# srsampson/SingleCarrier

Measured on NVIDIA B200. Metric: demodulated_msym_per_s, higher is better.
Workload: dtype f32

## Files before the change

### include/singlecarrier_b200.h

```cpp
#ifndef SINGLECARRIER_B200_H
#define SINGLECARRIER_B200_H

#include <stddef.h>
#include <stdint.h>

#ifdef __cplusplus
extern "C" {
#endif

#define SC_FRAME_SIZE        1880
#define SC_SYMBOLS_PER_FRAME 376
#define SC_PREAMBLE_LENGTH   128
#define SC_DATA_SYMBOLS      31
#define SC_BITS_PER_CALL     62
#define SC_NTAPS             49
#define SC_EQ_LENGTH         5
#define SC_PACKET_SYMBOLS    376

#define SC_OK        0
#define SC_EINVAL   -1
#define SC_ECUDA    -2
#define SC_ENOMEM   -3
#define SC_ESTATE   -4

// ... 8 lines not shown
    float    max_value;
    float    cost;
    int16_t  max_index;
    int16_t  matches;
    int16_t  rx_timing;
    uint8_t  valid;
    uint8_t  reserved0;
    uint32_t call_index;
    uint32_t reserved1;
} sc_frame_result;


int  sc_create(sc_modem **out, int device, int64_t n_streams, uint32_t flags, float foffset_hz);
void sc_destroy(sc_modem *m);
int  sc_reset(sc_modem *m);
int64_t  sc_n_streams(const sc_modem *m);
uint32_t sc_call_index(const sc_modem *m);
const char *sc_last_error(void);
const char *sc_version(void);
int  sc_device_count(void);
uint64_t sc_launch_count(void);

#define SC_OPT_SLAB_PARTS 1
#define SC_OPT_PROFILE    2
#define SC_OPT_H2D_MODE   3
#define SC_H2D_COLUMNS    0
#define SC_H2D_ROWS       1
#define SC_H2D_FULL       2
#define SC_H2D_COLUMNS_3D 3
#define SC_OPT_FE_SEARCH     4
#define SC_FE_SEARCH_DIRECT  0
#define SC_FE_SEARCH_MMA     1
#define SC_FE_SEARCH_TCGEN05 2
#define SC_OPT_TRACKER       5
#define SC_TRACKER_AUTO      0
#define SC_TRACKER_THREAD    1
#define SC_TRACKER_COOP      2
#define SC_TRACKER_COOP_MAX  1024
#define SC_OPT_OVERLAP       6
#define SC_OVERLAP_AUTO      0
#define SC_OVERLAP_OFF       1
#define SC_OVERLAP_ON        2
#define SC_OVERLAP_MAX       32768
int  sc_set_option(sc_modem *m, int option, int64_t value);
int  sc_profile_read(sc_modem *m, double out[4]);
int  sc_transfer_bytes(const sc_modem *m, uint64_t out[2]);
int  sc_release_caches(void);


int64_t sc_state_size(const sc_modem *m);
int  sc_state_export(sc_modem *m, void *buf, int64_t buf_bytes);
int  sc_state_import(sc_modem *m, const void *buf, int64_t buf_bytes);


int sc_rx_frames_dev(sc_modem *m, const int16_t *in, int64_t stream_stride, int n_frames,
                     sc_frame_result *results, int64_t result_stride, float *eq_dbg, void *stream);
int sc_rx_frames_host(sc_modem *m, const int16_t *in, int64_t stream_stride, int n_frames,
                      sc_frame_result *results, int64_t result_stride, float *eq_dbg);

int sc_rx_frames_soft_dev(sc_modem *m, const int16_t *in, int64_t stream_stride, int n_frames,
                          sc_frame_result *results, int64_t result_stride, float *symbols, void *stream);
int sc_rx_frames_soft_host(sc_modem *m, const int16_t *in, int64_t stream_stride, int n_frames,
                           sc_frame_result *results, int64_t result_stride, float *symbols);


typedef struct {
// ... 132 lines not shown
```

### singlecarrier_b200/csrc/sc_api.cu

```cuda
#include <math.h>
#include <stdarg.h>
#include <stdio.h>
#include <stdlib.h>
#include <string.h>

#include <algorithm>
#include <atomic>
#include <map>
#include <tuple>
#include <mutex>
#include <new>
#include <vector>

#include <nvtx3/nvToolsExt.h>

#include "sc_kernels.h"
#include "sc_common.cuh"

namespace sc {
std::atomic<unsigned long long> g_launch_count{0};
}

struct NvtxRange {
    explicit NvtxRange(const char *name) { nvtxRangePushA(name); }
// ... 58 lines not shown
    cudaEvent_t ev_tab1 = nullptr, ev_tab2 = nullptr;
    int tab_split = 0;
    std::vector<cudaEvent_t> ev_tabc;

    int16_t *stage_in[N_PIPE] = {};
    sc_frame_result *stage_res[N_PIPE] = {};
    float *stage_eq[N_PIPE] = {};
    float *stage_sym[N_PIPE] = {};
    size_t stage_in_cap = 0, stage_res_cap = 0, stage_eq_cap = 0, stage_sym_cap = 0;

    bool packet = false;
    int16_t *pk_hist2 = nullptr;
    float2 *pk_mix_hist2 = nullptr;
    int *pk_t_before[N_PIPE] = {}, *pk_t_at[N_PIPE] = {};
    int2 *pk_list[N_PIPE] = {};
    int *pk_count[N_PIPE] = {};
    float2 *pk_sym[N_PIPE] = {};
    cudaStream_t pk_stream[N_PIPE] = {};
    cudaEvent_t pk_ev_go[N_PIPE] = {}, pk_ev_done[N_PIPE] = {};
    size_t pk_slab_cap = 0;
    unsigned long long *pk_n_host_dev = nullptr;
    sc_packet_result *pk_stage = nullptr;
    size_t pk_stage_cap = 0;
    float2 *pk_sym_stage = nullptr;
    size_t pk_sym_stage_cap = 0;
    PacketKey pk_key;

    bool poisoned = false;
    bool in_flight = false;
    uint64_t h2d_bytes = 0, d2h_bytes = 0;

    int h2d_mode = SC_H2D_COLUMNS;
    const void *search_a_table = nullptr;
    bool fe_search_mma = false;
    bool fe_search_umma = false;
    const void *search_umma_master = nullptr;
    int slab_parts = 0;
    bool profile = false;
    int tracker = SC_TRACKER_AUTO;

    int overlap = SC_OVERLAP_AUTO;
    float2 *ov_win[OV_RING] = {};
    int *ov_max_index[OV_RING] = {};
    float *ov_max_value[OV_RING] = {};
    float *ov_state[OV_RING] = {};
    int *ov_timing[OV_RING] = {};
    cudaStream_t ov_stream[N_PIPE] = {}, ov_data[N_PIPE][2] = {};
    cudaEvent_t ov_ev_fe[N_PIPE][OV_RING] = {}, ov_ev_train[N_PIPE][OV_RING] = {}, ov_ev_data[N_PIPE][OV_RING] = {};
    cudaEvent_t ov_ev_first[N_PIPE] = {}, ov_join[N_PIPE][3] = {};
    bool ov_ready = false;
    std::vector<cudaEvent_t> ev_fe, ev_tk;
};

static inline unsigned lfsr_step(uint16_t &m) {
    unsigned out = ((m >> 1) ^ m) & 1u;
    m = (uint16_t) ((m >> 1) | (out << 14));
    return out;
}
static uint64_t keystream_next_word(uint16_t &m) {
    uint64_t w = 0;
    for (int j = 0; j < SC_BITS_PER_CALL; j++) w |= (uint64_t) lfsr_step(m) << j;
    return w;
}

static uint16_t lfsr_at_call(uint32_t call_index) {
    uint16_t m = 0x4A80;
    const uint32_t steps = (uint32_t) (((uint64_t) call_index * SC_BITS_PER_CALL) % 32767u);
    for (uint32_t k = 0; k < steps; k++) lfsr_step(m);
// ... 72 lines not shown
    if (const char *e = getenv("SC_OVERLAP")) m->overlap = std::max(0, std::min(atoi(e), (int) SC_OVERLAP_ON));
    m->rx_rect = nco_rect(-1100.0f + foffset_hz);
    m->tx_rect = nco_rect(1100.0f);
    int rc = SC_OK;
    auto body = [&]() -> int {
        CU(cudaSetDevice(device));
        const int64_t np = m->n_pad;
        CU(cudaMalloc(&m->timing[0], np * sizeof(int)));
        CU(cudaMalloc(&m->timing[1], np * sizeof(int)));
        CU(cudaMalloc(&m->timing_cold, np * sizeof(int)));
        {
            std::vector<int> t(np, 3);
            CU(cudaMemcpy(m->timing_cold, t.data(), np * sizeof(int), cudaMemcpyHostToDevice));
        }
        CU(cudaMalloc(&m->win, (size_t) (np / 32) * WIN_ROWS * 32 * sizeof(float2)));
        CU(cudaMalloc(&m->max_index, np * sizeof(int)));
        CU(cudaMalloc(&m->max_value, np * sizeof(float)));
        CU(cudaMalloc(&m->hist, (size_t) m->n * FRAME * sizeof(int16_t)));
        CU(cudaMemset(m->hist, 0, (size_t) m->n * FRAME * sizeof(int16_t)));
        CU(cudaMalloc(&m->rx_phase, sizeof(float2)));
        if (m->packet) {
            CU(cudaMalloc(&m->pk_hist2, (size_t) m->n * FRAME * sizeof(int16_t)));
            CU(cudaMemset(m->pk_hist2, 0, (size_t) m->n * FRAME * sizeof(int16_t)));
            CU(cudaMalloc(&m->pk_mix_hist2, (size_t) FRAME * sizeof(float2)));
            CU(cudaMemset(m->pk_mix_hist2, 0, (size_t) FRAME * sizeof(float2)));
            CU(cudaMalloc(&m->pk_n_host_dev, sizeof(unsigned long long)));
        }
        CU(cudaMalloc(&m->unit_phase, sizeof(float2)));
        {
            const float2 one = make_float2(1.0f, 0.0f);
            CU(cudaMemcpy(m->unit_phase, &one, sizeof one, cudaMemcpyHostToDevice));
        }
        if (const char *e = getenv("SC_FE_SEARCH")) {
            m->fe_search_umma = strcmp(e, "tcgen05") == 0;
            m->fe_search_mma = m->fe_search_umma || strcmp(e, "mma") == 0;
        }
        if (const char *e = getenv("SC_H2D_MODE")) m->h2d_mode = std::max(0, std::min(atoi(e), (int) SC_H2D_COLUMNS_3D));
        for (int i = 0; i < N_PIPE; i++) {
            CU(cudaStreamCreateWithFlags(&m->pipe[i], cudaStreamNonBlocking));
            CU(cudaEventCreateWithFlags(&m->ev_done[i], cudaEventDisableTiming));
        }
        CU(cudaEventCreateWithFlags(&m->ev_start, cudaEventDisableTiming));
        CU(cudaStreamCreateWithFlags(&m->tab_stream, cudaStreamNonBlocking));
        CU(cudaEventCreateWithFlags(&m->ev_tab1, cudaEventDisableTiming));
        CU(cudaEventCreateWithFlags(&m->ev_tab2, cudaEventDisableTiming));
        return modem_cold(m);
    };
    rc = body();
    if (rc != SC_OK) {
        sc_destroy(m);
        return rc;
    }
    *out = m;
    return SC_OK;
}

extern "C" void sc_destroy(sc_modem *m) {
    if (!m) return;
    cudaSetDevice(m->device);
    cudaDeviceSynchronize();
    cudaFree(m->timing[0]);
    cudaFree(m->timing[1]);
    cudaFree(m->timing_cold);
    for (cudaEvent_t e : m->ev_fe) cudaEventDestroy(e);
    for (cudaEvent_t e : m->ev_tk) cudaEventDestroy(e);
    cudaFree(m->win);
    cudaFree(m->max_index);
    cudaFree(m->max_value);
// ... 319 lines not shown
        CU(cudaMemcpy2DAsync(m->hist + (size_t) s0 * FRAME, FRAME * sizeof(int16_t), in + (size_t) (n_frames - 1) * FRAME,
                             (size_t) stride * sizeof(int16_t), FRAME * sizeof(int16_t), (size_t) ns, cudaMemcpyDeviceToDevice, st));
    return SC_OK;
}

static int run_slab(sc_modem *m, cudaStream_t st, int64_t s0, int ns, const int16_t *in, int64_t stride,
                    int n_frames, uint32_t call0, const uint64_t *kw, const float2 *mix0, int slot0,
                    sc_frame_result *results, int64_t result_stride, float *eq_dbg, float *sym, bool save_hist,
                    const PacketSink *pk = nullptr, int pipe = 0) {
    float2 *win = m->win + (size_t) (s0 / 32) * WIN_ROWS * 32;
    int tab_waited = -1;
    PacketSrc psrc;
    int pk_chunk = 0, pk_done = 0;
    if (pk) {
        if (ns > PK_CAP) return fail(SC_ESTATE, "packet mode: slab larger than the packet scratch");
        CU(cudaMemcpyAsync(m->pk_t_before[pipe], m->timing[(call0 + 1) & 1] + s0, (size_t) ns * sizeof(int), cudaMemcpyDeviceToDevice, st));
        CU(cudaMemcpyAsync(m->pk_t_at[pipe], m->timing[call0 & 1] + s0, (size_t) ns * sizeof(int), cudaMemcpyDeviceToDevice, st));
        psrc.results = results;
        psrc.result_stride = result_stride;
        psrc.in = in;
        psrc.stride = stride;
        psrc.hist1 = m->hist + (size_t) s0 * FRAME;
        psrc.hist2 = m->pk_hist2 + (size_t) s0 * FRAME;
        psrc.mix0 = mix0;
        psrc.mix_hist2 = slot0 >= 1 ? mix0 - FRAME : m->pk_mix_hist2;
        psrc.timing_before_call0 = m->pk_t_before[pipe];
        psrc.timing_at_call0 = m->pk_t_at[pipe];
        psrc.call0 = call0;
        psrc.stream0 = (int) s0;
        psrc.wide = m->wide;
        pk_chunk = std::max(1, PK_CAP / ns);
    }
    const bool tracker_coop = m->tracker == SC_TRACKER_COOP || (m->tracker == SC_TRACKER_AUTO && ns <= SC_TRACKER_COOP_MAX);
    const bool plain = !pk && !m->packet && !m->profile && !m->fe_search_mma && !eq_dbg && !m->state_dbg;
    if (plain && n_frames >= 2 && (m->overlap == SC_OVERLAP_ON || (m->overlap == SC_OVERLAP_AUTO && m->n <= SC_OVERLAP_MAX)))
        return run_slab_overlapped(m, st, pipe, s0, ns, in, stride, n_frames, call0, kw, mix0, slot0, results, result_stride,
                                   sym, save_hist, tracker_coop);
    for (int j = 0; j < n_frames; j++) {
        const uint32_t n = call0 + (uint32_t) j;
        int *tc = m->timing[n & 1] + s0, *tn = m->timing[(n + 1) & 1] + s0;
        if (m->profile) CU(prof_mark(m->ev_tk, st));
        {
            NvtxRange range("sc:track_kernel");
            CU(launch_track(m->debug_eq && eq_dbg != nullptr, win, m->max_index + s0, m->max_value + s0, tc, tn,
                            results + j, result_stride, eq_dbg ? eq_dbg + (size_t) j * 10 : nullptr,
                            m->state_dbg ? m->state_dbg + (size_t) s0 * TRACK_STATE_FLOATS : nullptr, n, kw[j], ns, st, tracker_coop,
                            sym ? sym + (size_t) j * SYM_FLOATS : nullptr));
        }
        if (m->profile) CU(prof_mark(m->ev_tk, st));
        if (n >= 1) {
            const int16_t *frame;
            int64_t fstride;
            if (j >= 1) {
                frame = in + (size_t) (j - 1) * FRAME;
                fstride = stride;
            } else {
                frame = m->hist + (size_t) s0 * FRAME;
                fstride = FRAME;
            }
            int rcw = table_wait(m, st, slot0 + j, tab_waited);
            if (rcw != SC_OK) return rcw;
            if (m->profile) CU(prof_mark(m->ev_fe, st));
            {
                NvtxRange range("sc:frontend_kernel");
                if (m->fe_search_umma && frontend_umma_eligible(frame, fstride))
                    CU(launch_frontend_umma(m->wide, frame, fstride, mix0 + (size_t) j * FRAME, tc, tn, win, m->max_index + s0,
                                            m->max_value + s0, ns, st, m->search_umma_master));
                else
                    CU(launch_frontend(m->wide, frame, fstride, mix0 + (size_t) j * FRAME, tc, tn, win, m->max_index + s0,
                                       m->max_value + s0, ns, st,
                                       m->fe_search_mma && !m->fe_search_umma ? m->search_a_table : nullptr));
            }
            if (m->profile) CU(prof_mark(m->ev_fe, st));
        }
        if (pk && (j + 1 - pk_done == pk_chunk || j + 1 == n_frames)) {
            NvtxRange range("sc:packet_pass");
            int rcw = table_wait(m, st, slot0 + j, tab_waited);
            if (rcw != SC_OK) return rcw;
            CU(cudaEventRecord(m->pk_ev_go[pipe], st));
            CU(cudaStreamWaitEvent(m->pk_stream[pipe], m->pk_ev_go[pipe], 0));
            CU(launch_packet_pass(psrc, ns, pk_done, j + 1, PK_CAP, m->pk_list[pipe], m->pk_count[pipe], m->pk_sym[pipe],
                                  m->pk_key, pk->packets, pk->capacity, pk->n_packets, pk->symbols, m->pk_stream[pipe]));
            pk_done = j + 1;
        }
    }
    if (pk) {
        CU(cudaEventRecord(m->pk_ev_done[pipe], m->pk_stream[pipe]));
        CU(cudaStreamWaitEvent(st, m->pk_ev_done[pipe], 0));
    }
    if (m->packet && save_hist && n_frames > 0) {
        if (n_frames >= 2)
            CU(cudaMemcpy2DAsync(m->pk_hist2 + (size_t) s0 * FRAME, FRAME * sizeof(int16_t),
                                 in + (size_t) (n_frames - 2) * FRAME, (size_t) stride * sizeof(int16_t),
                                 FRAME * sizeof(int16_t), (size_t) ns, cudaMemcpyDeviceToDevice, st));
        else
            CU(cudaMemcpyAsync(m->pk_hist2 + (size_t) s0 * FRAME, m->hist + (size_t) s0 * FRAME,
                               (size_t) ns * FRAME * sizeof(int16_t), cudaMemcpyDeviceToDevice, st));
    }
    if (save_hist && n_frames > 0) {
        CU(cudaMemcpy2DAsync(m->hist + (size_t) s0 * FRAME, FRAME * sizeof(int16_t),
                             in + (size_t) (n_frames - 1) * FRAME, (size_t) stride * sizeof(int16_t),
                             FRAME * sizeof(int16_t), (size_t) ns, cudaMemcpyDeviceToDevice, st));
    }
    return SC_OK;
}

static int64_t pick_slab(int64_t n, int64_t lo, int64_t parts) {
    int64_t s = (n + parts - 1) / parts;
    s = std::max<int64_t>(s, lo);
    s = (s + 127) / 128 * 128;
    return s;
}

static int rx_begin(sc_modem *m, const char *who, const int16_t *in, int64_t stream_stride, int n_frames,
                    sc_frame_result *results, int64_t result_stride, float *eq_dbg, std::vector<uint64_t> &kw,
                    uint16_t &lfsr) {
    if (!m || !in || !results || n_frames < 0) return fail(SC_EINVAL, "%s: bad arguments", who);
    if (m->poisoned) return fail(SC_ESTATE, "%s: an earlier batch failed part-way; call sc_reset() first", who);
    if (n_frames == 0) return SC_OK;
    if (stream_stride < (int64_t) n_frames * FRAME || result_stride < n_frames)
        return fail(SC_EINVAL, "%s: stride smaller than the batch", who);
    if (eq_dbg && !m->debug_eq) return fail(SC_EINVAL, "%s: eq_dbg needs SC_FLAG_DEBUG_EQ", who);
    if (m->fe_search_mma) {
        int rc = m->fe_search_umma ? search_umma_master(m->device, &m->search_umma_master)
                                   : search_table(m->device, &m->search_a_table);
        if (rc != SC_OK) return rc;
    }
    lfsr = m->lfsr_rx;
    kw.resize(n_frames);
    for (int j = 0; j < n_frames; j++) kw[j] = keystream_next_word(lfsr);
    return SC_OK;
}

static int rx_end(sc_modem *m, int rc, int n_frames, uint16_t lfsr) {
    if (rc != SC_OK) {
        if (m->in_flight) m->poisoned = true;
        m->in_flight = false;
        return rc;
    }
    m->in_flight = false;
    m->lfsr_rx = lfsr;
    m->call += (uint32_t) n_frames;
    return SC_OK;
}

static int rx_frames_dev_body(sc_modem *m, const int16_t *in, int64_t stream_stride, int n_frames,
                              sc_frame_result *results, int64_t result_stride, float *eq_dbg, float *sym,
                              cudaStream_t user, const uint64_t *kw, const PacketSink *pk = nullptr) {
    CU(cudaSetDevice(m->device));
    CU(cudaEventRecord(m->ev_start, user));
    CU(cudaStreamWaitEvent(m->pipe[0], m->ev_start, 0));
    m->in_flight = true;
    int rc = prepare_tables(m, n_frames, m->pipe[0]);
    if (rc != SC_OK) return rc;
    CU(cudaEventRecord(m->ev_start, m->pipe[0]));
    for (int i = 1; i < N_PIPE; i++) CU(cudaStreamWaitEvent(m->pipe[i], m->ev_start, 0));

    int64_t slab = pick_slab(m->n, m->slab_parts > 0 ? 128 : 8192, m->slab_parts > 0 ? m->slab_parts : 2);
    if (pk) slab = std::min<int64_t>(slab, PK_CAP);
    int k = 0;
// ... 879 lines not shown
    if (h.magic != STATE_MAGIC || h.version != STATE_VERSION) return fail(SC_EINVAL, "sc_state_import: not a state image");
    if (h.n != m->n || h.n_pad != m->n_pad || h.flags != m->flags || h.foffset != m->foffset)
        return fail(SC_EINVAL, "sc_state_import: the image was taken from a bank with other parameters");
    int rc = state_quiesce(m);
    if (rc != SC_OK) return rc;
    if (m->mix_cap < 1) {
        CU(cudaMalloc(&m->mix_table, (size_t) 2 * FRAME * sizeof(float2)));
        m->mix_cap = 1;
    }
    CU(cudaMemcpy(m->rx_phase, &h.rx_phase, sizeof(float2), cudaMemcpyHostToDevice));
    CU(cudaMemcpy(m->timing[h.call & 1], b + L.off_timing, (size_t) m->n_pad * sizeof(int), cudaMemcpyHostToDevice));
    CU(cudaMemcpy(m->max_index, b + L.off_maxi, (size_t) m->n_pad * sizeof(int), cudaMemcpyHostToDevice));
    CU(cudaMemcpy(m->max_value, b + L.off_maxv, (size_t) m->n_pad * sizeof(float), cudaMemcpyHostToDevice));
    CU(cudaMemcpy(m->win, b + L.off_win, (size_t) (m->n_pad / 32) * WIN_ROWS * 32 * sizeof(float2), cudaMemcpyHostToDevice));
    CU(cudaMemcpy(m->hist, b + L.off_hist, (size_t) m->n * FRAME * sizeof(int16_t), cudaMemcpyHostToDevice));
    CU(cudaMemcpy(m->mix_table, b + L.off_mix, (size_t) FRAME * sizeof(float2), cudaMemcpyHostToDevice));
    m->call = h.call;
    m->lfsr_rx = h.lfsr_rx;
    m->poisoned = m->in_flight = false;
    return SC_OK;
}

extern "C" int sc_set_option(sc_modem *m, int option, int64_t value) {
    if (!m) return fail(SC_EINVAL, "sc_set_option: null handle");
    switch (option) {
        case SC_OPT_SLAB_PARTS:
            if (value < 0 || value > 1024) return fail(SC_EINVAL, "sc_set_option: slab parts out of range");
            m->slab_parts = (int) value;
            return SC_OK;
        case SC_OPT_PROFILE:
            m->profile = value != 0;
            return SC_OK;
        case SC_OPT_FE_SEARCH:
            if (value != SC_FE_SEARCH_DIRECT && value != SC_FE_SEARCH_MMA && value != SC_FE_SEARCH_TCGEN05)
                return fail(SC_EINVAL, "sc_set_option: unknown search mode");
            m->fe_search_mma = value != SC_FE_SEARCH_DIRECT;
            m->fe_search_umma = value == SC_FE_SEARCH_TCGEN05;
            return SC_OK;
        case SC_OPT_TRACKER:
            if (value < SC_TRACKER_AUTO || value > SC_TRACKER_COOP) return fail(SC_EINVAL, "sc_set_option: unknown tracker");
            m->tracker = (int) value;
            return SC_OK;
        case SC_OPT_OVERLAP:
            if (value < SC_OVERLAP_AUTO || value > SC_OVERLAP_ON) return fail(SC_EINVAL, "sc_set_option: unknown overlap mode");
            m->overlap = (int) value;
            return SC_OK;
        case SC_OPT_H2D_MODE:
            if (value < SC_H2D_COLUMNS || value > SC_H2D_COLUMNS_3D) return fail(SC_EINVAL, "sc_set_option: unknown H2D mode");
            m->h2d_mode = (int) value;
            return SC_OK;
        default:
            return fail(SC_EINVAL, "sc_set_option: unknown option %d", option);
    }
}

static int prof_sum(std::vector<cudaEvent_t> &v, double *ms, double *count) {
    *ms = 0.0;
    *count = 0.0;
    for (size_t i = 0; i + 1 < v.size(); i += 2) {
        float t = 0.f;
        CU(cudaEventElapsedTime(&t, v[i], v[i + 1]));
        *ms += t;
        *count += 1.0;
    }
    for (cudaEvent_t e : v) cudaEventDestroy(e);
    v.clear();
    return SC_OK;
}

extern "C" int sc_profile_read(sc_modem *m, double out[4]) {
// ... 16 lines not shown
```

### singlecarrier_b200/csrc/sc_frontend_umma.cu

```cuda
#include "sc_common.cuh"
#include "sc_tables.cuh"
#include "sc_frontend.cuh"
#include "sc_umma.cuh"
#include "sc_kernels.h"

#include <stdio.h>
#include <stdlib.h>

namespace sc {

constexpr int FU_WIN = 16;
constexpr int FU_SRCH_WARP0 = FU_WIN, FU_SRCH_WARPS = 4;
constexpr int FU_THREADS = 32 * (FU_WIN + FU_SRCH_WARPS);
constexpr int FU_MIX_BYTES = FE_BUF * 8;
constexpr int FU_W_BYTES = WIN * 8;
static_assert(FU_W_BYTES % 128 == 16 && FU_MIX_BYTES % 16 == 0, "window stride");
constexpr int FU_N = 4 * FU_WIN;
constexpr int FU_KSTEPS = 2 * PRE / 16;
constexpr int FU_B_LBO = (FU_N / 8) * 128;
constexpr int FU_B_BYTES = (2 * PRE / 8) * FU_B_LBO;
constexpr int FU_SBO = 128;
constexpr int FU_A_LBO = ((SU_A_ROWS + 7) / 8) * 128;
constexpr int FU_A_BYTES = 2 * FU_A_LBO;
static_assert(FU_A_BYTES == 16 * SU_A_WORDS4 && FU_A_BYTES % 128 == 0, "master size");
constexpr int FU_TMEM_COLS = FU_N;
constexpr uint32_t FU_IDESC = (1u << 4) | (1u << 7) | (1u << 10) | ((uint32_t) (FU_N >> 3) << 17) | ((128u >> 4) << 24);

struct FuShared {
    unsigned long long a_full;
    unsigned long long tab_full;
    unsigned long long w_full;
    unsigned long long w_empty;
    unsigned long long mma_done;
    uint32_t tmem_base;
    uint32_t warp_max[FU_SRCH_WARPS][FU_WIN];
    float s_abs[FU_WIN];
    int maxidx[FU_WIN];
    int t2[FU_WIN];
    int n_cand[FU_SRCH_WARPS][FU_WIN];
    float ver_v[FU_SRCH_WARPS][FU_WIN];
    int ver_i[FU_SRCH_WARPS][FU_WIN];
    unsigned char cand[FU_SRCH_WARPS][FU_WIN][SM_MAX_CAND];
};
constexpr int FU_OFF_B = FU_A_BYTES;
constexpr int FU_OFF_W = FU_OFF_B + FU_B_BYTES;
constexpr int FU_OFF_MIX = FU_OFF_W + FU_WIN * FU_W_BYTES;
constexpr int FU_TAB_BYTES = FRAME * 8;
constexpr int FU_OFF_TAB = FU_OFF_MIX + FU_WIN * FU_MIX_BYTES;
constexpr int FU_OFF_CTRL = FU_OFF_TAB + FU_TAB_BYTES;
static_assert(FU_OFF_TAB % 16 == 0 && FU_TAB_BYTES % 16 == 0, "TMA bulk copy of the table");
static_assert(FU_OFF_B % 128 == 0 && FU_OFF_W % 128 == 0 && FU_OFF_MIX % 16 == 0 && FU_OFF_CTRL % 16 == 0, "alignment");
constexpr int FU_SMEM = FU_OFF_CTRL + (int) sizeof(FuShared) + 1024;
static_assert(FU_SMEM <= 227 * 1024, "one CTA per SM");

__device__ __forceinline__ void umma_bf16_ss(uint32_t tmem_d, uint64_t a_desc, uint64_t b_desc, uint32_t accumulate) {
    asm volatile(
        "{\n\t.reg .pred p;\n\t"
        "setp.ne.b32 p, %4, 0;\n\t"
        "tcgen05.mma.cta_group::1.kind::f16 [%0], %1, %2, %3, p;\n\t}" ::"r"(tmem_d),
        "l"(a_desc), "l"(b_desc), "r"(FU_IDESC), "r"(accumulate)
        : "memory");
}
__device__ __forceinline__ void fu_tmem_ld16(uint32_t taddr, float (&v)[16]) {
    uint32_t r[16];
    asm volatile(
        "tcgen05.ld.sync.aligned.32x32b.x16.b32 {%0, %1, %2, %3, %4, %5, %6, %7, %8, %9, %10, %11, %12, %13, %14, %15}, [%16];"
        : "=r"(r[0]), "=r"(r[1]), "=r"(r[2]), "=r"(r[3]), "=r"(r[4]), "=r"(r[5]), "=r"(r[6]), "=r"(r[7]), "=r"(r[8]),
          "=r"(r[9]), "=r"(r[10]), "=r"(r[11]), "=r"(r[12]), "=r"(r[13]), "=r"(r[14]), "=r"(r[15])
        : "r"(taddr));
#pragma unroll
    for (int i = 0; i < 16; i++) v[i] = __uint_as_float(r[i]);
}
__device__ __forceinline__ void srch_bar() { asm volatile("bar.sync 1, 128;" ::: "memory"); }

#ifdef FU_PROFILE
#define FU_T(acc) { const long long t_ = clock64(); acc += t_ - t_last; t_last = t_; }
#else
#define FU_T(acc)
#endif

__device__ __forceinline__ int ld_pinned(const int *p) {
    int v;
    asm volatile("ld.global.nc.b32 %0, [%1];" : "=r"(v) : "l"(p));
    return v;
}

template <bool WIDE>
__global__ void __launch_bounds__(FU_THREADS, 1)
frontend_umma_kernel(const int16_t *__restrict__ in, long stream_stride, const float2 *__restrict__ mix_table,
                     const int *__restrict__ timing_cur, const int *__restrict__ timing_next,
                     float2 *__restrict__ win, int *__restrict__ max_index_out, float *__restrict__ max_value_out,
                     int n_streams, const uint4 *__restrict__ a_master) {
    extern __shared__ unsigned char fu_smem_raw[];
    unsigned char *fu_smem = fu_smem_raw + ((1024u - (smem_u32(fu_smem_raw) & 1023u)) & 1023u);
    unsigned char *sA = fu_smem;
    unsigned char *sB = fu_smem + FU_OFF_B;
    unsigned char *sW = fu_smem + FU_OFF_W;
    FuShared &sh = *reinterpret_cast<FuShared *>(fu_smem + FU_OFF_CTRL);

    const int tid = threadIdx.x, warp = tid >> 5, lane = tid & 31;
    const long n_batches = ((long) n_streams + FU_WIN - 1) / FU_WIN;
    const long my_batches = blockIdx.x < n_batches ? (n_batches - blockIdx.x + gridDim.x - 1) / gridDim.x : 0;

    if (tid == 0) {
        mbar_init(&sh.a_full, 1);
        mbar_init(&sh.tab_full, 1);
        mbar_init(&sh.w_full, FU_WIN);
        mbar_init(&sh.w_empty, FU_SRCH_WARPS);
        mbar_init(&sh.mma_done, 1);
        asm volatile("fence.mbarrier_init.release.cluster;" ::: "memory");
    }
    if (warp == FU_SRCH_WARP0) {
        asm volatile("tcgen05.alloc.cta_group::1.sync.aligned.shared::cta.b32 [%0], %1;" ::"r"(smem_u32(&sh.tmem_base)),
                     "r"((uint32_t) FU_TMEM_COLS)
                     : "memory");
        asm volatile("tcgen05.relinquish_alloc_permit.cta_group::1.sync.aligned;" ::: "memory");
    }
    tc_fence_before();
    __syncthreads();
    tc_fence_after();
    if (tid == 0) {
        mbar_expect_tx(&sh.a_full, (uint32_t) FU_A_BYTES);
        tma_bulk_g2s(sA, a_master, (uint32_t) FU_A_BYTES, &sh.a_full);
        mbar_expect_tx(&sh.tab_full, (uint32_t) FU_TAB_BYTES);
        tma_bulk_g2s(fu_smem + FU_OFF_TAB, mix_table, (uint32_t) FU_TAB_BYTES, &sh.tab_full);
    }
    const uint32_t tmem = sh.tmem_base;
#ifdef FU_PROFILE
    long long t_last = clock64(), p0 = 0, p1 = 0, p2 = 0, p3 = 0, p4 = 0, p5 = 0, p6 = 0, p7 = 0;
    const long long t_begin = t_last;
#endif

    if (warp < FU_WIN) {
        float2 *mix = reinterpret_cast<float2 *>(fu_smem + FU_OFF_MIX + warp * FU_MIX_BYTES);
        float2 *W = reinterpret_cast<float2 *>(sW + warp * FU_W_BYTES);
        auto stream_of = [&](long n) { return (blockIdx.x + n * gridDim.x) * FU_WIN + warp; };
        int shift = 0, base2 = 0;
        const float2 *const tab_s = reinterpret_cast<const float2 *>(fu_smem + FU_OFF_TAB);
        const float2 *tab = tab_s;
        const uint32_t *fp = nullptr;
        uint32_t raw[FE_KN];
#pragma unroll
        for (int k = 0; k < FE_KN; k++) raw[k] = 0u;
        auto setup = [&](long sx, int T) {
            const int base = max(min(T, 2 * PRE - 1) - (NTAPS - 1), 0);
            base2 = base & ~1;
            shift = base - base2;
            fp = reinterpret_cast<const uint32_t *>(in + sx * stream_stride + base2);
            tab = tab_s + base2;
        };
        long s = stream_of(0);
        bool active = my_batches > 0 && s < n_streams;
        if (active) {
            setup(s, ld_pinned(timing_cur + s));
            fe_load<FE_KA_LO>(raw, fp, lane, base2);
        }
        long s_nx = stream_of(1);
        bool act_nx = my_batches > 1 && s_nx < n_streams;
        int T_nx = act_nx ? ld_pinned(timing_cur + s_nx) : 0;
        mbar_wait(&sh.tab_full, 0u);
#pragma unroll 1
        for (long n = 0; n < my_batches; n++) {
            const int t2 = active ? ld_pinned(timing_next + s) : 0;
            u64 accA[FE_R], accB[FE_R];
            {
                const int front = FE_FRONT + (shift & 1);
                if (active) {
                    fe_stage<FE_KA_LO, true>(mix, raw, tab, lane, front - shift);
                    fe_load<FE_KB_LO>(raw, fp, lane, base2);
                }
                __syncwarp();
#pragma unroll
                for (int r = 0; r < FE_R; r++) accA[r] = 0ull;
                if (active && lane < FE_FIR_LANES) fe_fir<WIDE>(mix, front, lane, accA);
                __syncwarp();
            }
            {
                constexpr int h0 = CYC * FE_PASS_OUT;
                const int front = FE_FRONT + ((shift + h0) & 1);
                if (active) fe_stage<FE_KB_LO, true>(mix, raw, tab, lane, front - shift - h0);
                const bool active_cur = active;
                s = s_nx;
                active = act_nx;
                if (active) {
                    setup(s, T_nx);
                    fe_load<FE_KA_LO>(raw, fp, lane, base2);
                }
                s_nx = stream_of(n + 2);
                act_nx = n + 2 < my_batches && s_nx < n_streams;
                T_nx = act_nx ? ld_pinned(timing_cur + s_nx) : 0;
                __syncwarp();
#pragma unroll
                for (int r = 0; r < FE_R; r++) accB[r] = 0ull;
                if (active_cur && lane < FE_FIR_LANES) fe_fir<WIDE>(mix, front, lane, accB);
                __syncwarp();
            }
            FU_T(p0)
            mbar_wait(&sh.w_empty, ((uint32_t) n & 1u) ^ 1u);
            FU_T(p1)
            float part = 0.0f;
            if (lane < FE_FIR_LANES) {
#pragma unroll
                for (int r = 0; r < FE_R; r++) {
                    float yr, yi;
                    unpk(accA[r], yr, yi);
                    const float2 wa = make_float2(__fmul_rn(yr, FIR_GAIN), __fmul_rn(yi, FIR_GAIN));
                    unpk(accB[r], yr, yi);
                    const float2 wb = make_float2(__fmul_rn(yr, FIR_GAIN), __fmul_rn(yi, FIR_GAIN));
                    const int xa = FE_R * lane + r, xb = FE_PASS_OUT + xa;
                    W[xa] = wa;
                    W[xb] = wb;
                    part = __fadd_rn(part, __fadd_rn(fabsf(__fsub_rn(wa.x, wa.y)), fabsf(__fadd_rn(wa.y, wa.x))));
                    if (xb < SEARCH_SYMS)
                        part = __fadd_rn(part, __fadd_rn(fabsf(__fsub_rn(wb.x, wb.y)), fabsf(__fadd_rn(wb.y, wb.x))));
                }
            }
#pragma unroll
            for (int off = 16; off > 0; off >>= 1) part = __fadd_rn(part, __shfl_xor_sync(0xffffffffu, part, off));
            if (lane == 0) {
                sh.s_abs[warp] = part;
                sh.t2[warp] = t2;
            }
            __syncwarp();
            if (lane == 0) mbar_arrive(&sh.w_full);
            FU_T(p2)
        }
    } else {
        const int q4 = warp - FU_SRCH_WARP0, st = tid - 32 * FU_SRCH_WARP0, lag = st;
#pragma unroll 1
        for (long n = 0; n < my_batches; n++) {
            const long s0 = (blockIdx.x + n * gridDim.x) * FU_WIN;
            const uint32_t ph = (uint32_t) n & 1u;
            mbar_wait_relaxed(&sh.w_full, ph);
            FU_T(p0)
#pragma unroll 1
            for (int i = 0; i < 4; i++) {
                const int w = st & 15, c = 8 * i + (st >> 4);
                const uint4 *src = reinterpret_cast<const uint4 *>(sW + w * FU_W_BYTES + c * 64);
                uint32_t dh[4], dm[4], eh[4], em[4];
#pragma unroll
                for (int q = 0; q < 4; q++) {
                    const uint4 v = src[q];
                    float d0 = __fsub_rn(__uint_as_float(v.x), __uint_as_float(v.y));
                    float e0 = __fadd_rn(__uint_as_float(v.y), __uint_as_float(v.x));
                    float d1 = __fsub_rn(__uint_as_float(v.z), __uint_as_float(v.w));
                    float e1 = __fadd_rn(__uint_as_float(v.w), __uint_as_float(v.z));
                    if (c == 31 && q == 3) d1 = e1 = 0.0f;
                    split2_pair(d0, d1, dh[q], dm[q]);
                    split2_pair(e0, e1, eh[q], em[q]);
                }
                unsigned char *dst = sB + c * FU_B_LBO + (w >> 3) * 128 + (w & 7) * 16;
                *reinterpret_cast<uint4 *>(dst + 0 * 256) = make_uint4(dh[0], dh[1], dh[2], dh[3]);
                *reinterpret_cast<uint4 *>(dst + 1 * 256) = make_uint4(dm[0], dm[1], dm[2], dm[3]);
                *reinterpret_cast<uint4 *>(dst + 2 * 256) = make_uint4(eh[0], eh[1], eh[2], eh[3]);
                *reinterpret_cast<uint4 *>(dst + 3 * 256) = make_uint4(em[0], em[1], em[2], em[3]);
            }
            asm volatile("fence.proxy.async.shared::cta;" ::: "memory");
            tc_fence_before();
            srch_bar();
            FU_T(p1)

// ... 240 lines not shown
```

### singlecarrier_b200/modem.py

```python
from __future__ import annotations

import ctypes as C
from typing import Optional

import numpy as np

from ._lib import SC_FLAG_DEBUG_EQ, SC_FLAG_PACKET, SC_FLAG_WIDE, Channel, check, lib

FRAME_SIZE = 1880
SYMBOLS_PER_FRAME = 376
BITS_PER_CALL = 62
DATA_SYMBOLS = 31
PACKET_FRAMES = 8
PACKET_DATA_SYMBOLS = PACKET_FRAMES * DATA_SYMBOLS
PACKET_SAMPLES = 1880
OPT_SLAB_PARTS, OPT_PROFILE, OPT_H2D_MODE, OPT_FE_SEARCH, OPT_TRACKER, OPT_OVERLAP = 1, 2, 3, 4, 5, 6
OVERLAP_AUTO, OVERLAP_OFF, OVERLAP_ON, OVERLAP_MAX = 0, 1, 2, 32768
TRACKER_AUTO, TRACKER_THREAD, TRACKER_COOP, TRACKER_COOP_MAX = 0, 1, 2, 1024
FE_SEARCH_DIRECT, FE_SEARCH_MMA, FE_SEARCH_TCGEN05 = 0, 1, 2
H2D_COLUMNS, H2D_ROWS, H2D_FULL, H2D_COLUMNS_3D = 0, 1, 2, 3
N_COUNTERS, N_BER_COUNTERS, N_PACKET_BER_COUNTERS = 16, 8, 32
REFERENCE_GAP = 903

RESULT_DTYPE = np.dtype([("bits", "<u8"), ("max_value", "<f4"), ("cost", "<f4"), ("max_index", "<i2"),
                         ("matches", "<i2"), ("rx_timing", "<i2"), ("valid", "u1"), ("reserved0", "u1"),
                         ("call_index", "<u4"), ("reserved1", "<u4")])
assert RESULT_DTYPE.itemsize == 32
PACKET_DTYPE = np.dtype([("bits", "<u8", (8,)), ("stream", "<i4"), ("call_index", "<u4"), ("max_index", "<i2"),
                         ("matches", "<i2"), ("cost", "<f4"), ("reserved0", "<u4"), ("reserved1", "<u4"),
                         ("reserved2", "<u8")])
assert PACKET_DTYPE.itemsize == 96


def keystream_word(call_index: int) -> int:
    return int(lib.sc_keystream_word(call_index))


def soft_bits(results: np.ndarray, symbols: np.ndarray) -> np.ndarray:
    r = np.asarray(results)
    assert r.dtype == RESULT_DTYPE
    sym = np.asarray(symbols, np.complex64)
    assert sym.shape == r.shape + (DATA_SYMBOLS,)
    soft = np.empty(r.shape + (BITS_PER_CALL,), np.float32)
    soft[..., 0::2] = sym.imag
    soft[..., 1::2] = sym.real
    calls = r["call_index"].ravel()
    uniq, inv = np.unique(calls, return_inverse=True)
    words = np.array([keystream_word(int(c)) for c in uniq], np.uint64)[inv].reshape(r.shape)
    flip = ((words[..., None] >> np.arange(BITS_PER_CALL, dtype=np.uint64)) & np.uint64(1)).astype(bool)
    soft[flip] = -soft[flip]
    return soft

# ... 294 lines not shown
```

Baseline: 66300.

## Rework tcgen05 frontend FIR warps and auto-select it for large slabs

Restructures the tcgen05 frontend so 11 FIR warps round-robin over the 16 frames of each batch. Each warp computes the whole 290-sample window in one pass with 10 outputs per lane instead of two half-passes, which shrinks the shared-memory mix buffers. Adds an AUTO search mode as the new default that picks the tcgen05 path when the slab has at least 16384 streams. The aim is fewer FIR passes and less shared memory per block, at the cost of more registers per lane and a different warp-to-frame mapping that has to keep the mbarrier accounting correct.

```diff
diff --git a/include/singlecarrier_b200.h b/include/singlecarrier_b200.h
--- a/include/singlecarrier_b200.h
+++ b/include/singlecarrier_b200.h
@@ -64,6 +64,8 @@
 #define SC_FE_SEARCH_DIRECT  0
 #define SC_FE_SEARCH_MMA     1
 #define SC_FE_SEARCH_TCGEN05 2
+#define SC_FE_SEARCH_AUTO    3
+#define SC_FE_TCGEN05_MIN_SLAB 16384
 #define SC_OPT_TRACKER       5
 #define SC_TRACKER_AUTO      0
 #define SC_TRACKER_THREAD    1
diff --git a/singlecarrier_b200/csrc/sc_api.cu b/singlecarrier_b200/csrc/sc_api.cu
--- a/singlecarrier_b200/csrc/sc_api.cu
+++ b/singlecarrier_b200/csrc/sc_api.cu
@@ -114,8 +114,7 @@
 
     int h2d_mode = SC_H2D_COLUMNS;
     const void *search_a_table = nullptr;
-    bool fe_search_mma = false;
-    bool fe_search_umma = false;
+    int fe_search = SC_FE_SEARCH_AUTO;
     const void *search_umma_master = nullptr;
     int slab_parts = 0;
     bool profile = false;
@@ -254,8 +253,10 @@
             CU(cudaMemcpy(m->unit_phase, &one, sizeof one, cudaMemcpyHostToDevice));
         }
         if (const char *e = getenv("SC_FE_SEARCH")) {
-            m->fe_search_umma = strcmp(e, "tcgen05") == 0;
-            m->fe_search_mma = m->fe_search_umma || strcmp(e, "mma") == 0;
+            m->fe_search = strcmp(e, "tcgen05") == 0 ? SC_FE_SEARCH_TCGEN05
+                         : strcmp(e, "mma") == 0     ? SC_FE_SEARCH_MMA
+                         : strcmp(e, "auto") == 0    ? SC_FE_SEARCH_AUTO
+                                                     : SC_FE_SEARCH_DIRECT;
         }
         if (const char *e = getenv("SC_H2D_MODE")) m->h2d_mode = std::max(0, std::min(atoi(e), (int) SC_H2D_COLUMNS_3D));
         for (int i = 0; i < N_PIPE; i++) {
@@ -641,10 +642,12 @@
         pk_chunk = std::max(1, PK_CAP / ns);
     }
     const bool tracker_coop = m->tracker == SC_TRACKER_COOP || (m->tracker == SC_TRACKER_AUTO && ns <= SC_TRACKER_COOP_MAX);
-    const bool plain = !pk && !m->packet && !m->profile && !m->fe_search_mma && !eq_dbg && !m->state_dbg;
+    const bool fe_forced = m->fe_search == SC_FE_SEARCH_MMA || m->fe_search == SC_FE_SEARCH_TCGEN05;
+    const bool plain = !pk && !m->packet && !m->profile && !fe_forced && !eq_dbg && !m->state_dbg;
     if (plain && n_frames >= 2 && (m->overlap == SC_OVERLAP_ON || (m->overlap == SC_OVERLAP_AUTO && m->n <= SC_OVERLAP_MAX)))
         return run_slab_overlapped(m, st, pipe, s0, ns, in, stride, n_frames, call0, kw, mix0, slot0, results, result_stride,
                                    sym, save_hist, tracker_coop);
+    const bool fe_umma = m->fe_search == SC_FE_SEARCH_TCGEN05 || (m->fe_search == SC_FE_SEARCH_AUTO && ns >= SC_FE_TCGEN05_MIN_SLAB);
     for (int j = 0; j < n_frames; j++) {
         const uint32_t n = call0 + (uint32_t) j;
         int *tc = m->timing[n & 1] + s0, *tn = m->timing[(n + 1) & 1] + s0;
@@ -672,13 +675,13 @@
             if (m->profile) CU(prof_mark(m->ev_fe, st));
             {
                 NvtxRange range("sc:frontend_kernel");
-                if (m->fe_search_umma && frontend_umma_eligible(frame, fstride))
+                if (fe_umma && frontend_umma_eligible(frame, fstride))
                     CU(launch_frontend_umma(m->wide, frame, fstride, mix0 + (size_t) j * FRAME, tc, tn, win, m->max_index + s0,
                                             m->max_value + s0, ns, st, m->search_umma_master));
                 else
                     CU(launch_frontend(m->wide, frame, fstride, mix0 + (size_t) j * FRAME, tc, tn, win, m->max_index + s0,
                                        m->max_value + s0, ns, st,
-                                       m->fe_search_mma && !m->fe_search_umma ? m->search_a_table : nullptr));
+                                       m->fe_search == SC_FE_SEARCH_MMA ? m->search_a_table : nullptr));
             }
             if (m->profile) CU(prof_mark(m->ev_fe, st));
         }
@@ -730,11 +733,12 @@
     if (stream_stride < (int64_t) n_frames * FRAME || result_stride < n_frames)
         return fail(SC_EINVAL, "%s: stride smaller than the batch", who);
     if (eq_dbg && !m->debug_eq) return fail(SC_EINVAL, "%s: eq_dbg needs SC_FLAG_DEBUG_EQ", who);
-    if (m->fe_search_mma) {
-        int rc = m->fe_search_umma ? search_umma_master(m->device, &m->search_umma_master)
-                                   : search_table(m->device, &m->search_a_table);
-        if (rc != SC_OK) return rc;
-    }
+    int rc = SC_OK;
+    if (m->fe_search == SC_FE_SEARCH_TCGEN05 || (m->fe_search == SC_FE_SEARCH_AUTO && m->n >= SC_FE_TCGEN05_MIN_SLAB))
+        rc = search_umma_master(m->device, &m->search_umma_master);
+    else if (m->fe_search == SC_FE_SEARCH_MMA)
+        rc = search_table(m->device, &m->search_a_table);
+    if (rc != SC_OK) return rc;
     lfsr = m->lfsr_rx;
     kw.resize(n_frames);
     for (int j = 0; j < n_frames; j++) kw[j] = keystream_next_word(lfsr);
@@ -1680,10 +1684,8 @@
             m->profile = value != 0;
             return SC_OK;
         case SC_OPT_FE_SEARCH:
-            if (value != SC_FE_SEARCH_DIRECT && value != SC_FE_SEARCH_MMA && value != SC_FE_SEARCH_TCGEN05)
-                return fail(SC_EINVAL, "sc_set_option: unknown search mode");
-            m->fe_search_mma = value != SC_FE_SEARCH_DIRECT;
-            m->fe_search_umma = value == SC_FE_SEARCH_TCGEN05;
+            if (value < SC_FE_SEARCH_DIRECT || value > SC_FE_SEARCH_AUTO) return fail(SC_EINVAL, "sc_set_option: unknown search mode");
+            m->fe_search = (int) value;
             return SC_OK;
         case SC_OPT_TRACKER:
             if (value < SC_TRACKER_AUTO || value > SC_TRACKER_COOP) return fail(SC_EINVAL, "sc_set_option: unknown tracker");
diff --git a/singlecarrier_b200/csrc/sc_frontend_umma.cu b/singlecarrier_b200/csrc/sc_frontend_umma.cu
--- a/singlecarrier_b200/csrc/sc_frontend_umma.cu
+++ b/singlecarrier_b200/csrc/sc_frontend_umma.cu
@@ -10,9 +10,18 @@
 namespace sc {
 
 constexpr int FU_WIN = 16;
-constexpr int FU_SRCH_WARP0 = FU_WIN, FU_SRCH_WARPS = 4;
-constexpr int FU_THREADS = 32 * (FU_WIN + FU_SRCH_WARPS);
-constexpr int FU_MIX_BYTES = FE_BUF * 8;
+constexpr int FU_FIR_WARPS = 11;
+constexpr int FU_SRCH_WARP0 = FU_FIR_WARPS, FU_SRCH_WARPS = 4;
+static_assert(FU_FIR_WARPS <= FU_WIN, "every FIR warp has a frame in every batch (one w_empty wait per batch)");
+constexpr int FU_THREADS = 32 * (FU_FIR_WARPS + FU_SRCH_WARPS);
+constexpr int FU_R = 10;
+constexpr int FU_FIR_LANES = WIN / FU_R;
+constexpr int FU_FIR_SAMP = NTAPS + CYC * (FU_R - 1);
+constexpr int FU_NROUND = FE_PAIRS_PER_LANE;
+static_assert(FU_FIR_LANES * FU_R == WIN, "290 = 29 x 10");
+constexpr int FU_BUF = FE_FRONT + 2 * FE_NPAIR + 2;
+static_assert(FE_FRONT + CYC * FU_R * (FU_FIR_LANES - 1) + FU_FIR_SAMP + 1 <= FU_BUF && FE_FRONT % 2 == 0, "FIR reads");
+constexpr int FU_MIX_BYTES = FU_BUF * 8;
 constexpr int FU_W_BYTES = WIN * 8;
 static_assert(FU_W_BYTES % 128 == 16 && FU_MIX_BYTES % 16 == 0, "window stride");
 constexpr int FU_N = 4 * FU_WIN;
@@ -46,7 +55,7 @@
 constexpr int FU_OFF_W = FU_OFF_B + FU_B_BYTES;
 constexpr int FU_OFF_MIX = FU_OFF_W + FU_WIN * FU_W_BYTES;
 constexpr int FU_TAB_BYTES = FRAME * 8;
-constexpr int FU_OFF_TAB = FU_OFF_MIX + FU_WIN * FU_MIX_BYTES;
+constexpr int FU_OFF_TAB = FU_OFF_MIX + FU_FIR_WARPS * FU_MIX_BYTES;
 constexpr int FU_OFF_CTRL = FU_OFF_TAB + FU_TAB_BYTES;
 static_assert(FU_OFF_TAB % 16 == 0 && FU_TAB_BYTES % 16 == 0, "TMA bulk copy of the table");
 static_assert(FU_OFF_B % 128 == 0 && FU_OFF_W % 128 == 0 && FU_OFF_MIX % 16 == 0 && FU_OFF_CTRL % 16 == 0, "alignment");
@@ -83,6 +92,49 @@
     int v;
     asm volatile("ld.global.nc.b32 %0, [%1];" : "=r"(v) : "l"(p));
     return v;
+}
+
+__device__ __forceinline__ void fu_load(uint32_t (&raw)[FU_NROUND], const uint32_t *__restrict__ fp, int lane) {
+#pragma unroll
+    for (int k = 0; k < FU_NROUND; k++) {
+        const int p = lane + 32 * k;
+        raw[k] = k < FU_NROUND - 1 || p < FE_NPAIR ? __ldg(fp + p) : 0u;
+    }
+}
+
+__device__ __forceinline__ void fu_stage(float2 *__restrict__ buf, const uint32_t (&raw)[FU_NROUND],
+                                         const float2 *__restrict__ tab, int lane) {
+#pragma unroll
+    for (int k = 0; k < FU_NROUND; k++) {
+        const int p = lane + 32 * k;
+        if (k < FU_NROUND - 1 || p < FE_NPAIR) {
+            const float4 ph = *reinterpret_cast<const float4 *>(tab + 2 * p);
+            const float v0 = (float) (int16_t) (raw[k] & 0xffffu);
+            const float v1 = (float) (int16_t) (raw[k] >> 16);
+            *reinterpret_cast<float4 *>(buf + FE_FRONT + 2 * p) = make_float4(__fmul_rn(ph.x, v0), __fmul_rn(ph.y, v0),
+                                                                              __fmul_rn(ph.z, v1), __fmul_rn(ph.w, v1));
+        }
+    }
+}
+
+template <bool WIDE, int ODD>
+__device__ __forceinline__ void fu_fir(const float2 *__restrict__ buf, int lane, u64 (&acc)[FU_R]) {
+    const ulonglong2 *mp = reinterpret_cast<const ulonglong2 *>(buf + FE_FRONT + CYC * FU_R * lane);
+#pragma unroll
+    for (int m = 0; m < (FU_FIR_SAMP + ODD + 1) / 2; m++) {
+        const ulonglong2 v = mp[m];
+#pragma unroll
+        for (int e = 0; e < 2; e++) {
+            const int j = 2 * m + e - ODD;
+            if (j < 0 || j >= FU_FIR_SAMP) continue;
+            const u64 x = e ? v.y : v.x;
+#pragma unroll
+            for (int r = 0; r < FU_R; r++) {
+                const int k = j - CYC * r;
+                if (k >= 0 && k < NTAPS) acc[r] = pk_add(acc[r], pk_mul_bcast_pz(x, tap<WIDE>(k)));
+            }
+        }
+    }
 }
 
 template <bool WIDE>
@@ -131,102 +183,100 @@
     const long long t_begin = t_last;
 #endif
 
-    if (warp < FU_WIN) {
+    if (warp < FU_FIR_WARPS) {
         float2 *mix = reinterpret_cast<float2 *>(fu_smem + FU_OFF_MIX + warp * FU_MIX_BYTES);
-        float2 *W = reinterpret_cast<float2 *>(sW + warp * FU_W_BYTES);
-        auto stream_of = [&](long n) { return (blockIdx.x + n * gridDim.x) * FU_WIN + warp; };
-        int shift = 0, base2 = 0;
+        const long my_frames = (my_batches * FU_WIN - warp + FU_FIR_WARPS - 1) / FU_FIR_WARPS;
+        auto stream_of = [&](long i) {
+            const long g = warp + FU_FIR_WARPS * i;
+            return (blockIdx.x + (g / FU_WIN) * gridDim.x) * FU_WIN + g % FU_WIN;
+        };
+        long n_waited = -1;
+        int shift = 0;
         const float2 *const tab_s = reinterpret_cast<const float2 *>(fu_smem + FU_OFF_TAB);
         const float2 *tab = tab_s;
         const uint32_t *fp = nullptr;
-        uint32_t raw[FE_KN];
-#pragma unroll
-        for (int k = 0; k < FE_KN; k++) raw[k] = 0u;
+        uint32_t raw[FU_NROUND];
+#pragma unroll
+        for (int k = 0; k < FU_NROUND; k++) raw[k] = 0u;
         auto setup = [&](long sx, int T) {
             const int base = max(min(T, 2 * PRE - 1) - (NTAPS - 1), 0);
-            base2 = base & ~1;
+            const int base2 = base & ~1;
             shift = base - base2;
             fp = reinterpret_cast<const uint32_t *>(in + sx * stream_stride + base2);
             tab = tab_s + base2;
         };
         long s = stream_of(0);
-        bool active = my_batches > 0 && s < n_streams;
+        bool active = my_frames > 0 && s < n_streams;
         if (active) {
             setup(s, ld_pinned(timing_cur + s));
-            fe_load<FE_KA_LO>(raw, fp, lane, base2);
+            fu_load(raw, fp, lane);
         }
         long s_nx = stream_of(1);
-        bool act_nx = my_batches > 1 && s_nx < n_streams;
+        bool act_nx = my_frames > 1 && s_nx < n_streams;
         int T_nx = act_nx ? ld_pinned(timing_cur + s_nx) : 0;
         mbar_wait(&sh.tab_full, 0u);
 #pragma unroll 1
-        for (long n = 0; n < my_batches; n++) {
+        for (long f = 0; f < my_frames; f++) {
+            const long g = warp + FU_FIR_WARPS * f, n = g / FU_WIN;
+            const int w = (int) (g % FU_WIN);
             const int t2 = active ? ld_pinned(timing_next + s) : 0;
-            u64 accA[FE_R], accB[FE_R];
-            {
-                const int front = FE_FRONT + (shift & 1);
-                if (active) {
-                    fe_stage<FE_KA_LO, true>(mix, raw, tab, lane, front - shift);
-                    fe_load<FE_KB_LO>(raw, fp, lane, base2);
-                }
-                __syncwarp();
-#pragma unroll
-                for (int r = 0; r < FE_R; r++) accA[r] = 0ull;
-                if (active && lane < FE_FIR_LANES) fe_fir<WIDE>(mix, front, lane, accA);
-                __syncwarp();
-            }
-            {
-                constexpr int h0 = CYC * FE_PASS_OUT;
-                const int front = FE_FRONT + ((shift + h0) & 1);
-                if (active) fe_stage<FE_KB_LO, true>(mix, raw, tab, lane, front - shift - h0);
-                const bool active_cur = active;
-                s = s_nx;
-                active = act_nx;
-                if (active) {
-                    setup(s, T_nx);
-                    fe_load<FE_KA_LO>(raw, fp, lane, base2);
-                }
-                s_nx = stream_of(n + 2);
-                act_nx = n + 2 < my_batches && s_nx < n_streams;
-                T_nx = act_nx ? ld_pinned(timing_cur + s_nx) : 0;
-                __syncwarp();
-#pragma unroll
-                for (int r = 0; r < FE_R; r++) accB[r] = 0ull;
-                if (active_cur && lane < FE_FIR_LANES) fe_fir<WIDE>(mix, front, lane, accB);
-                __syncwarp();
-            }
+            if (active) fu_stage(mix, raw, tab, lane);
+            const bool active_cur = active;
+            const int odd = shift;
+            s = s_nx;
+            active = act_nx;
+            if (active) {
+                setup(s, T_nx);
+                fu_load(raw, fp, lane);
+            }
+            s_nx = stream_of(f + 2);
+            act_nx = f + 2 < my_frames && s_nx < n_streams;
+            T_nx = act_nx ? ld_pinned(timing_cur + s_nx) : 0;
+            __syncwarp();
+            u64 acc[FU_R];
+#pragma unroll
+            for (int r = 0; r < FU_R; r++) acc[r] = 0ull;
+            if (active_cur && lane < FU_FIR_LANES) {
+                if (odd) fu_fir<WIDE, 1>(mix, lane, acc);
+                else fu_fir<WIDE, 0>(mix, lane, acc);
+            }
+            __syncwarp();
             FU_T(p0)
-            mbar_wait(&sh.w_empty, ((uint32_t) n & 1u) ^ 1u);
+            if (n != n_waited) {
+                mbar_wait(&sh.w_empty, ((uint32_t) n & 1u) ^ 1u);
+                n_waited = n;
+            }
             FU_T(p1)
+            float2 *W = reinterpret_cast<float2 *>(sW + w * FU_W_BYTES);
             float part = 0.0f;
-            if (lane < FE_FIR_LANES) {
-#pragma unroll
-                for (int r = 0; r < FE_R; r++) {
+            if (lane < FU_FIR_LANES) {
+#pragma unroll
+                for (int r = 0; r < FU_R; r += 2) {
                     float yr, yi;
-                    unpk(accA[r], yr, yi);
+                    unpk(acc[r], yr, yi);
                     const float2 wa = make_float2(__fmul_rn(yr, FIR_GAIN), __fmul_rn(yi, FIR_GAIN));
-                    unpk(accB[r], yr, yi);
+                    unpk(acc[r + 1], yr, yi);
                     const float2 wb = make_float2(__fmul_rn(yr, FIR_GAIN), __fmul_rn(yi, FIR_GAIN));
-                    const int xa = FE_R * lane + r, xb = FE_PASS_OUT + xa;
-                    W[xa] = wa;
-                    W[xb] = wb;
-                    part = __fadd_rn(part, __fadd_rn(fabsf(__fsub_rn(wa.x, wa.y)), fabsf(__fadd_rn(wa.y, wa.x))));
-                    if (xb < SEARCH_SYMS)
+                    const int x = FU_R * lane + r;
+                    *reinterpret_cast<float4 *>(W + x) = make_float4(wa.x, wa.y, wb.x, wb.y);
+                    if (x < SEARCH_SYMS)
+                        part = __fadd_rn(part, __fadd_rn(fabsf(__fsub_rn(wa.x, wa.y)), fabsf(__fadd_rn(wa.y, wa.x))));
+                    if (x + 1 < SEARCH_SYMS)
                         part = __fadd_rn(part, __fadd_rn(fabsf(__fsub_rn(wb.x, wb.y)), fabsf(__fadd_rn(wb.y, wb.x))));
                 }
             }
 #pragma unroll
             for (int off = 16; off > 0; off >>= 1) part = __fadd_rn(part, __shfl_xor_sync(0xffffffffu, part, off));
             if (lane == 0) {
-                sh.s_abs[warp] = part;
-                sh.t2[warp] = t2;
+                sh.s_abs[w] = part;
+                sh.t2[w] = t2;
             }
             __syncwarp();
             if (lane == 0) mbar_arrive(&sh.w_full);
             FU_T(p2)
         }
     } else {
-        const int q4 = warp - FU_SRCH_WARP0, st = tid - 32 * FU_SRCH_WARP0, lag = st;
+        const int q4 = warp & 3, st = 32 * q4 + lane, lag = st;
 #pragma unroll 1
         for (long n = 0; n < my_batches; n++) {
             const long s0 = (blockIdx.x + n * gridDim.x) * FU_WIN;
diff --git a/singlecarrier_b200/modem.py b/singlecarrier_b200/modem.py
--- a/singlecarrier_b200/modem.py
+++ b/singlecarrier_b200/modem.py
@@ -17,7 +17,8 @@
 OPT_SLAB_PARTS, OPT_PROFILE, OPT_H2D_MODE, OPT_FE_SEARCH, OPT_TRACKER, OPT_OVERLAP = 1, 2, 3, 4, 5, 6
 OVERLAP_AUTO, OVERLAP_OFF, OVERLAP_ON, OVERLAP_MAX = 0, 1, 2, 32768
 TRACKER_AUTO, TRACKER_THREAD, TRACKER_COOP, TRACKER_COOP_MAX = 0, 1, 2, 1024
-FE_SEARCH_DIRECT, FE_SEARCH_MMA, FE_SEARCH_TCGEN05 = 0, 1, 2
+FE_SEARCH_DIRECT, FE_SEARCH_MMA, FE_SEARCH_TCGEN05, FE_SEARCH_AUTO = 0, 1, 2, 3
+FE_TCGEN05_MIN_SLAB = 16384
 H2D_COLUMNS, H2D_ROWS, H2D_FULL, H2D_COLUMNS_3D = 0, 1, 2, 3
 N_COUNTERS, N_BER_COUNTERS, N_PACKET_BER_COUNTERS = 16, 8, 32
 REFERENCE_GAP = 903
```

Measured after the change: 55130 (median of 6 runs). 16.8% lower.
